# datasciencetoolkit/NextGP.jl

Measured on AMD Instinct MI355X. Metric: gibbs_iterations_per_sec, higher is better.
Workload: dtype f64; 1 GPU; single-trait Gibbs sweep, N=50000 individuals x P=600000 SNPs, marker sets BayesPR(200000) + BayesPR(200000) + BayesPR(200000), fp32 panel in HBM (BASELINE.json configs[3]: multi-breed random regression = three BayesPR marker sets of 200,000 SNPs); N=50000, P=600000, chains=1, panel_dtype=f32, accumulate_dtype=f64

## Files before the change

### nextgp.jl_amd/csrc/ngp_sweep.h

```cpp
#pragma once
#include <cstddef>
#include <type_traits>
#include "ngp_sweep_args.h"

#ifndef NGP_ROWS_DPP
#define NGP_ROWS_DPP 1
#endif

#pragma clang fp contract(off)

namespace ngp {


#define NGP_DBG_FOLD                                                     \
    unsigned long long *const dbg = DBG ? A.dbg : nullptr;               \
    const int dbg_mode = DBG ? A.dbg_mode : 0;                           \
    (void)dbg; (void)dbg_mode;
#define NGP_DBG_LOCALS                                                   \
    unsigned long long *const dbg = A.dbg;                               \
    const int dbg_mode = A.dbg_mode;                                     \
    (void)dbg; (void)dbg_mode;
#define NGP_DBG_ROWS NGP_DBG_FOLD

__device__ inline unsigned ld_u32(const unsigned *p) { return __hip_atomic_load(p, __ATOMIC_RELAXED, __HIP_MEMORY_SCOPE_AGENT); }
// ... 1051 lines not shown
                        red[(par * NGP_ROWS_NW + wv) * NGP_BLK + lane] = acc;
                        asm volatile("" ::: "memory");
                        if (lane == 0) __hip_atomic_fetch_add((lds_int_t *)(par ? gcnt1 : gcnt0), 1, __ATOMIC_RELAXED, __HIP_MEMORY_SCOPE_WORKGROUP);
                        try_signal(false);
                        const char *tq = ring + (size_t)wrap(base + tslot) * NGP_QS + c * 128;
#pragma unroll
                        for (int jj = 0; jj < 8; jj++) keep[d][hh][jj] = *(const float4 *)(tq + jj * 16);
                    }
                    if (wv == NGP_ROWS_PUBW && u < nb) {
                        const int *gc = par ? gcnt1 : gcnt0;
                        for (unsigned sp = 0; lds_flag_ld(gc) < NGP_ROWS_NW; ++sp) {
                            if ((sp & 255u) == 255u && (lds_flag_ld(sflag) == 0 || sp > (NGP_SPIN_LIMIT << 4))) {
                                if (lane == 0) *sflag = 0;
                                break;
                            }
                            __builtin_amdgcn_s_sleep(0);
                        }
                        asm volatile("" ::: "memory");
                        if (lane == 0) lds_flag_st(par ? gcnt0 : gcnt1, 0);
                        publish(u, hh, par);
                    }
                    if (pollw) {
                        int ok = 1;
                        if (!have_dnext) {
                            ok = wait_dlt_granules_all(A.dltg, A.nonce, pa, lane, A.abort_w, 1u, pg0, pg1) ? 1 : 0;
                            if (!ok && lane == 0) *sflag = 0;
                        }
                        if (ok) dl[((u + 1) & 1) * NGP_DLS + lane] = dlt_granules_value(pg0, pg1);
                    }
                    if (wv == NGP_ROWS_POLLW && hh == V - 1 && pa + 1 >= 0 && u + 2 < nb + DT) {
                        const unsigned long long *gp = A.dltg + ((size_t)((pa + 1) % NGP_RING) * NGP_BLK + lane) * 2;
                        pg0 = ld_u64(gp);
                        pg1 = ld_u64(gp + 1);
                    }
                    try_signal(DT < 4 || (A.knob & 16));
                    wg_barrier();
                    if (!*sflag) return;
                    base = wrap(base + NQ);
                }
            }
        }
        try_signal(true);
    }
    __syncthreads();
    for (int i = tid; i < V * R; i += NGP_WG) yg[i] = ys[(i / R) * RP + (i % R)];
}

template <bool DBG>
__device__ __attribute__((always_inline)) inline void role_reducer(const SweepArgs &A, const int g, char *smem, const int wv0 = 0,
                                                                   const int nwv = NGP_WG / 64) {
    NGP_DBG_LOCALS
    const int tid = threadIdx.x, wv = tid >> 6, lane = tid & 63;
    const int nb = A.t1 - A.t0;
    if (A.near + 1 + g >= A.D) return;
    const double fxs = A.scal->fx_scale;
    for (int u = wv - wv0; u < nb; u += nwv) {
        const int slot = u % NGP_RING;
        for (int d = A.near + 1 + g; d < A.D; d += A.NG) {
            const int a = u - d;
            if (a < 0) continue;
            double gr[NGP_BLK];
            load_rows_pair(A.gramx + ((size_t)(A.t0 + u) * A.D + d) * (NGP_BLK * NGP_BLK), lane, gr);
            unsigned long long q0, q1;
            {
                const unsigned long long *gp = A.dltg + ((size_t)(a % NGP_RING) * NGP_BLK + lane) * 2;
                q0 = ld_u64(gp);
                q1 = ld_u64(gp + 1);
            }
            if (!(dbg_mode == 3 || dbg_mode == 4 || dbg_mode == 6) && !wait_dlt_granules_all(A.dltg, A.nonce, a, lane, A.abort_w, 4u, q0, q1)) return;
            const double dreg = dlt_granules_value(q0, q1);
            double *ldw = (double *)smem + (size_t)wv * NGP_BLK;
            ldw[lane] = dreg;
            typedef const __attribute__((address_space(3))) double *lds_cdp;
            const lds_cdp dk = (lds_cdp)ldw;
            double s0 = 0.0, s1 = 0.0, s2 = 0.0, s3 = 0.0;
#pragma unroll
            for (int kk = 0; kk < NGP_BLK; kk += 16) {
                double dv[16];
#pragma unroll
                for (int i = 0; i < 16; i++) dv[i] = dk[kk + i];
#pragma unroll
                for (int i = 0; i < 16; i += 4) {
                    s0 = __builtin_fma(gr[kk + i + 0], dv[i + 0], s0);
                    s1 = __builtin_fma(gr[kk + i + 1], dv[i + 1], s1);
                    s2 = __builtin_fma(gr[kk + i + 2], dv[i + 2], s2);
                    s3 = __builtin_fma(gr[kk + i + 3], dv[i + 3], s3);
                }
                asm volatile("" : "+v"(s0), "+v"(s1), "+v"(s2), "+v"(s3));
            }
            const double v = (s0 + s1) + (s2 + s3);
            acc_add(A.acc, A.abort_w, slot, d, lane, -v, fxs);
            if (dbg && g == 0 && lane == 0) dbg[NGP_DBG_RED + 2 * (size_t)u + 1] = wall_clock64();
        }
    }
}

struct CoefRegs {
    double bo, cc, ww, st, gd;
    unsigned tf;
};
__device__ inline CoefRegs load_coef(const SweepArgs &A, long long k) {
    CoefRegs c;
    c.bo = A.beta[k];
    c.cc = A.c[k];
    c.ww = A.w[k];
    c.st = A.q[k];
    c.gd = A.mpm[k];
    c.tf = A.lin_all ? 1u : (A.blin ? A.blin[k >> 6] : 0u);
    return c;
}
__device__ __attribute__((always_inline)) inline unsigned acc_terms(const SweepArgs &A, const int u) {
    const int nfar = max(0, min(A.D - 1, u) - A.near);
    return (unsigned)(A.S + nfar);
}
__device__ __attribute__((always_inline)) inline unsigned long long acc_load(const SweepArgs &A, const int u, const int j) {
    const unsigned long long *ap = A.acc + (size_t)(u % NGP_RING) * NGP_FX_COPIES * NGP_BLK + j;
    unsigned long long qv[NGP_FX_COPIES];
#pragma unroll
    for (int c = 0; c < NGP_FX_COPIES; c++) qv[c] = ld_u64(ap + (size_t)c * NGP_BLK);
    unsigned long long q = qv[0];
#pragma unroll
    for (int c = 1; c < NGP_FX_COPIES; c++) q += qv[c];
    return q;
}
__device__ __attribute__((always_inline)) inline bool acc_complete(const unsigned long long q, const unsigned terms) {
    return __ballot((unsigned)(q & ((1ull << NGP_FX_CNT_BITS) - 1ull)) == terms) == ~0ull;
}
__device__ __attribute__((always_inline)) inline double acc_take(const SweepArgs &A, const int u, const int j, const unsigned long long q, const double fxi) {
    unsigned long long *ap = A.acc + (size_t)(u % NGP_RING) * NGP_FX_COPIES * NGP_BLK + j;
#pragma unroll
    for (int c = 0; c < NGP_FX_COPIES; c++) st_u64(ap + (size_t)c * NGP_BLK, 0ull);
    return fx_to_f64((long long)q >> NGP_FX_CNT_BITS) * fxi;
}
template <bool DBG, bool NGBIG = false>
__device__ __attribute__((always_inline)) inline bool fetch_group_sums(const SweepArgs &A, int u, int j, double *tot_out) {
    NGP_DBG_LOCALS
    const unsigned terms = acc_terms(A, u);
    const double fxi = A.scal->fx_inv;
    for (unsigned spins = 0;; ++spins) {
        const unsigned long long q = acc_load(A, u, j);
        if (dbg_mode == 2 || acc_complete(q, terms)) {
            *tot_out = acc_take(A, u, j, q, fxi);
            return true;
        }
        if ((spins & 7u) == 7u && ld_u32(A.abort_w) != 0u) return false;
        if (spins > (NGP_SPIN_LIMIT >> 3)) {
            st_u32(A.abort_w, 3u);
            return false;
        }
        __builtin_amdgcn_s_sleep(2);
    }
}

template <bool DBG>
__device__ __attribute__((always_inline)) inline void publish_block(const SweepArgs &A, int up, int j, const double *hist, const double *outb, const int *outi,
                                     const int *smeth, const double *ssdf) {
    NGP_DBG_LOCALS
    const int pbuf = up & 1;
    (void)hist;
    const long long k = (long long)(A.t0 + up) * NGP_BLK + j;
    const int si = A.setof[k];
    const double chik = A.chi[k];
    const int vbi = A.vbidx[k];
    st_f64(&A.dlt[(size_t)(up % NGP_RING) * NGP_BLK + j], hist[(up % NGP_RING) * NGP_BLK + j]);
    drain_vm();
    if (j == 0) st_u32(A.flag_dlt, (unsigned)(up + 1));
    if (dbg && j == 0) dbg[4 * (size_t)up + 2] = wall_clock64();
    const double bn = outb[pbuf * NGP_BLK + j];
    const int isave = outi[pbuf * NGP_BLK + j];
    A.beta[k] = bn;
    A.delta[k] = (uint8_t)isave;
    const int meth = (si >= 0) ? smeth[si] : -1;
    if (meth == 1) {
        double vb = 0.0;
        if (isave) {
            double tt = ssdf[si];
            double b2 = bn * bn;
            tt = tt + b2;
            vb = tt / chik;
            atomicAdd(&A.sets[si].nloci, 1);
        }
        A.varBeta[vbi] = vb;
    } else if (meth == 2) {
        if (isave) atomicAdd(&A.sets[si].nloci, 1);
    } else if (meth == 3) {
        atomicAdd(&A.sets[si].ncls[isave - 1], 1);
    }
}

struct RWide { double dmine; int c; };
__device__ __attribute__((noinline)) RWide rform_search_wide(const double *rcls, const size_t Ppad, const size_t col, const int j, const int Kk,
                                                             const double qv, const double av, const double tv, const double uv,
                                                             const double hs_k, const double rhs_k, const double bo_k) {
    const bool on = j < Kk;
    double q2 = qv, a2 = av, t2 = tv, u2 = uv;
    if (j >= NGP_RLDS && on) {
        const double *gp = rcls + (size_t)j * Ppad + col;
        const size_t gstr = (size_t)NGP_RMAX * Ppad;
        q2 = gp[0]; a2 = gp[gstr]; t2 = gp[2 * gstr]; u2 = gp[3 * gstr];
    }
    const double Lv = (q2 == 0.0) ? a2 : __builtin_fma(hs_k, q2, a2);
    RWide out;
    out.dmine = (q2 != 0.0) ? __builtin_fma(rhs_k, q2, t2) - bo_k : -bo_k;
    double m = readlane_d(Lv, 0);
#pragma unroll 1
    for (int v = 1; v < Kk; v++) {
        const double Lu = readlane_d(Lv, v);
        m = (Lu > m) ? Lu : m;
    }
    const double ev = on ? det_exp(Lv - m) : 0.0;
    double S = 0.0;
#pragma unroll 1
    for (int v = 0; v < Kk; v++) S = S + readlane_d(ev, v);
    int c = Kk - 1;
    double cum = 0.0;
#pragma unroll 1
    for (int v = 0; v < Kk; v++) {
        cum = cum + readlane_d(ev, v);
        const double thr = readlane_d(u2, v) * S;
        if (cum >= thr) { c = v; break; }
    }
    out.c = c;
    return out;
}

template <bool DBG, bool NGBIG = false, bool TUP = true, int RCLS = 1>
__device__ __attribute__((always_inline)) inline void role_sampler(const SweepArgs &A, char *smem) {
    NGP_DBG_LOCALS
    const int D = A.D, tid = threadIdx.x, wv = tid >> 6, j = tid & 63;
    double *Gd = (double *)smem;
    double *hist = Gd + 3 * 4096;
    double *vacc = hist + NGP_RING * NGP_BLK;
    double *r0 = vacc + NGP_RING * NGP_BLK;
    double *outb = r0 + 4 * NGP_BLK;
    int *outi = (int *)(outb + 2 * NGP_BLK);
    int *sabort = outi + 2 * NGP_BLK;
    int *totflag = sabort + 1;
    int *smeth = sabort + 4;
    double *ssdf = (double *)(sabort + 20);
    const int nb = A.t1 - A.t0;
    const size_t bsz = NGP_BLK * NGP_BLK;
    int *sK = sabort + 52;
    double *tl = (double *)(sabort + 80);
    int *tmeta = (int *)(tl + 2 * 9 * NGP_BLK);
    auto tuple_prefetch = [&](const int ub) __attribute__((always_inline)) {
        if (!TUP || !A.tup || ub >= nb) return;
        const long long tblk = (long long)(A.t0 + ub);
        const long long kcol = tblk * NGP_BLK + j;
        const int si = A.setof[kcol];
        const unsigned long long mask = __ballot(si >= 0 && smeth[si < 0 ? 0 : si] == NGP_METHOD_TUPLE_DEV);
        int *meta = tmeta + (ub & 1) * 4;
        if (mask == 0ull) {
            if (j == 0) meta[0] = 0;
            return;
        }
        const int sit = __builtin_amdgcn_readfirstlane(__shfl(si, __builtin_ctzll(mask)));
        const TupLane TL = load_tuplane(A.tupc, A.tupg, A.w, A.Ppad, kcol);
        const int k = A.tup[sit].k;
        const long long first_locus = (tblk - (A.tup[sit].col0 >> 6)) * tuple_loci_per_block(k);
        const int nvalid = tuple_nvalid(k, A.tup[sit].nloc, first_locus);
        double *dst = tl + (size_t)(ub & 1) * (9 * NGP_BLK) + j;
#pragma unroll
        for (int b = 0; b < NGP_KMAX; b++) { dst[b * NGP_BLK] = TL.crow[b]; dst[(NGP_KMAX + b) * NGP_BLK] = TL.grow[b]; }
        dst[2 * NGP_KMAX * NGP_BLK] = TL.ww;
        if (j == 0) { meta[0] = k; meta[1] = nvalid; }
    };
    double *rl = (double *)(tmeta + 16);
    int *rlm = (int *)(rl + 2 * 17 * NGP_BLK);
    int *rmeta = rlm + 2 * 128;
    double *rlx = (double *)(rmeta + 16);
    auto rcls_prefetch = [&](const int ub) __attribute__((always_inline)) {
        if (RCLS != 2 || !A.rcls || ub >= nb) return;
        const long long kcol = (long long)(A.t0 + ub) * NGP_BLK + j;
        const int si = A.setof[kcol];
        const int meth = (si >= 0) ? smeth[si] : -1;
        const int Kc = (si >= 0) ? sK[si] : 2;
        const unsigned long long mask = __ballot(meth == 3);
        if (j == 0) rmeta[(ub & 1) * 4] = (mask != 0ull) ? 1 : 0;
        if (mask == 0ull) return;
        RLane RL = empty_rlane();
        if (meth == 3) RL = load_rlane(A.rcls, A.Ppad, kcol, Kc, A.rhs0);
        double *dst = rl + (size_t)(ub & 1) * (17 * NGP_BLK) + j;
#pragma unroll
        for (int v = 0; v < NGP_RREG; v++) {
            dst[v * NGP_BLK] = RL.q[v]; dst[(4 + v) * NGP_BLK] = RL.a[v]; dst[(8 + v) * NGP_BLK] = RL.t[v]; dst[(12 + v) * NGP_BLK] = RL.u[v];
        }
        dst[16 * NGP_BLK] = RL.rhs0;
        rlm[(ub & 1) * 128 + j] = meth;
        rlm[(ub & 1) * 128 + 64 + j] = Kc;
        if (__ballot(meth == 3 && Kc > NGP_RREG) != 0ull) {
            double *dx = rlx + (size_t)(ub & 1) * (16 * NGP_BLK) + j;
#pragma unroll
            for (int arr = 0; arr < 4; arr++)
#pragma unroll
                for (int v = NGP_RREG; v < NGP_RLDS; v++) {
                    const bool on = (meth == 3) && v < Kc;
                    dx[(arr * 4 + v - NGP_RREG) * NGP_BLK] = on ? A.rcls[((size_t)arr * NGP_RMAX + v) * (size_t)A.Ppad + (size_t)kcol] : 0.0;
                }
        }
    };
    if (tid < 16) {
        smeth[tid] = A.sets[tid].method;
        ssdf[tid] = A.sets[tid].sdf;
        sK[tid] = A.sets[tid].K;
    }
    if (tid == 0) {
        *sabort = 0;
        *totflag = 0;
        st_u32(A.xcc_w, xcc_id() + 1u);
        if (dbg) { dbg[NGP_DBG_ALL - 2] = xcc_id(); dbg[NGP_DBG_ALL - 1] = (unsigned)__builtin_amdgcn_s_getreg((31 << 11) | 4); }
    }
    {
        const double *gd = chain_block_src(A, A.t0, A.lin_all || (A.blin && A.blin[A.t0] != 0u));
        for (int idx = tid; idx < 4096; idx += NGP_WG) Gd[idx] = gd[idx];
        if (nb > 1) {
            const double *gd1 = chain_block_src(A, A.t0 + 1, A.lin_all || (A.blin && A.blin[A.t0 + 1] != 0u));
            for (int idx = tid; idx < 4096; idx += NGP_WG) Gd[4096 + idx] = gd1[idx];
        }
    }
    __syncthreads();
    if (wv == 2) {
        double tot;
        if (fetch_group_sums<DBG, NGBIG>(A, 0, j, &tot)) r0[j] = tot;
        else if (j == 0) *sabort = 1;
    }
    if (wv == 1) { tuple_prefetch(0); rcls_prefetch(0); }
    __syncthreads();
    if (*sabort) return;
#define NGP_END_OF_BLOCK()                                                                       \
    do {                                                                                         \
        if (dbg && j == 0) dbg[NGP_DBG_WAVES + 8 * (size_t)u + wv] = wall_clock64();           \
        wg_barrier();                                                                            \
        if (*sabort) return;                                                                     \
    } while (0)
    if (wv == 0) {
        CoefRegs cur = load_coef(A, (long long)A.t0 * NGP_BLK + j), nxt = cur;
        double iVarE_sweep = 0.0;
        if constexpr (RCLS == 2) {
            if (A.rcls) iVarE_sweep = A.scal->iVarE;
        }
        for (int u = 0; u < nb; ++u) {
            const int t = A.t0 + u, buf = u & 1, slot = u % NGP_RING, rs = u & 3;
            if (dbg && j == 0) dbg[4 * (size_t)u] = wall_clock64();
            if (u + 1 < nb) nxt = load_coef(A, (long long)(t + 1) * NGP_BLK + j);
            constexpr bool PRELOAD = false;
            const bool tform = __builtin_amdgcn_readfirstlane((int)cur.tf) != 0;
            const double *gdb = Gd + (u % 3) * 4096 + j;
            double G[NGP_BLK];
            double tot;
            if (D == 1) {
                tot = r0[rs * NGP_BLK + j];
                bool okc = true;
                if (u >= 1) okc = fetch_group_sums<DBG, NGBIG>(A, u, j, &tot);
                if (!okc && j == 0) *sabort = 1;
            } else {
                for (unsigned sp = 0; lds_flag_ld(totflag) != u + 1; ++sp) {
                    if ((sp & 255u) == 255u && (lds_flag_ld(sabort) != 0 || sp > (NGP_SPIN_LIMIT << 4))) {
                        if (j == 0) *sabort = 1;
                        break;
                    }
                    __builtin_amdgcn_s_sleep(0);
                }
                asm volatile("" ::: "memory");
                tot = r0[rs * NGP_BLK + j];
            }
            if (DBG && dbg && j == 0) dbg[NGP_DBG_W5 + 4 * (size_t)u + 2] = wall_clock64();
            const double bo = cur.bo, cc = cur.cc, ww = cur.ww, st = cur.st;
            const double r = __builtin_fma(cur.gd, bo, tot);
#define NGP_LOAD_G()                                                           \
    if constexpr (!PRELOAD) { _Pragma("unroll") for (int kk = 0; kk < NGP_BLK; kk++) G[kk] = gdb[kk * NGP_BLK]; } \
    double H0 = -(cc * G[0]), H1 = -(cc * G[1]), H2 = -(cc * G[2]), H3 = -(cc * G[3]);
            double e = __builtin_fma(r, cc, ww);
            double dsave;
            int isave = 1;
            int meth0 = -1, si0 = -1, rblk = 0;
            if constexpr (RCLS == 1) {
                if (A.rcls) {
                    si0 = A.setof[(long long)t * NGP_BLK + j];
                    meth0 = (si0 >= 0) ? smeth[si0] : -1;
                }
            } else if constexpr (RCLS == 2) {
                if (A.rcls) rblk = __builtin_amdgcn_readfirstlane(rmeta[buf * 4]);
                if (rblk) meth0 = rlm[buf * 128 + j];
            }
            int tk = 0;
            if constexpr (TUP) {
                if (A.tup) tk = __builtin_amdgcn_readfirstlane(tmeta[buf * 4]);
            }
            if (tform && dbg_mode != 5) {
                double e0 = e;
                if constexpr (TUP) {
                    if (tk != 0) {
                        const int nvalid = __builtin_amdgcn_readfirstlane(tmeta[buf * 4 + 1]);
                        const double *tsrc = tl + (size_t)buf * (9 * NGP_BLK) + j;
                        TupLane TL;
#pragma unroll
                        for (int b = 0; b < NGP_KMAX; b++) { TL.crow[b] = tsrc[b * NGP_BLK]; TL.grow[b] = tsrc[(NGP_KMAX + b) * NGP_BLK]; }
                        TL.ww = tsrc[2 * NGP_KMAX * NGP_BLK];
                        e0 = tuple_e0(tk, nvalid, j, tot, bo, TL);
                    }
                }
                r0[rs * NGP_BLK + j] = e0;
                typedef const __attribute__((address_space(3))) double *lds_cdp;
                const lds_cdp ek = (lds_cdp)(r0 + rs * NGP_BLK);
                double s0 = 0.0, s1 = 0.0, s2 = 0.0, s3 = 0.0;
#pragma unroll
                for (int kk = 0; kk < NGP_BLK; kk += 16) {
                    double ev[16], tv[16];
#pragma unroll
                    for (int i = 0; i < 16; i++) ev[i] = ek[kk + i];
#pragma unroll
                    for (int i = 0; i < 16; i++) tv[i] = PRELOAD ? G[kk + i] : gdb[(kk + i) * NGP_BLK];
#pragma unroll
                    for (int i = 0; i < 16; i += 4) {
                        s0 = __builtin_fma(tv[i + 0], ev[i + 0], s0);
                        s1 = __builtin_fma(tv[i + 1], ev[i + 1], s1);
                        s2 = __builtin_fma(tv[i + 2], ev[i + 2], s2);
                        s3 = __builtin_fma(tv[i + 3], ev[i + 3], s3);
                    }
                    asm volatile("" : "+v"(s0), "+v"(s1), "+v"(s2), "+v"(s3));
                }
                dsave = (s0 + s1) + (s2 + s3);
                isave = 1;
            } else if (TUP && tk != 0) {
                const int nvalid = __builtin_amdgcn_readfirstlane(tmeta[buf * 4 + 1]);
                const double *tsrc = tl + (size_t)buf * (9 * NGP_BLK) + j;
                TupLane TL;
#pragma unroll
                for (int b = 0; b < NGP_KMAX; b++) { TL.crow[b] = tsrc[b * NGP_BLK]; TL.grow[b] = tsrc[(NGP_KMAX + b) * NGP_BLK]; }
                TL.ww = tsrc[2 * NGP_KMAX * NGP_BLK];
                dsave = tuple_chain_nv(tk, nvalid, j, tot, bo, TL, [&](int sl, int cc2) { return Gd[(u % 3) * 4096 + sl * NGP_BLK + cc2]; });
                isave = 1;
            } else if (RCLS != 0 && A.rcls && (RCLS == 2 ? rblk != 0 : __ballot(meth0 == 3) != 0ull)) {
                double dfin = 0.0;
                int cfin = 1;
                if constexpr (RCLS == 2) {
                    const double *cq = rl + (size_t)buf * (17 * NGP_BLK);
                    const double *cx = rlx + (size_t)buf * (16 * NGP_BLK);
                    const bool isr = (meth0 == 3);
                    const double q0j = cq[j], hstar = (isr && q0j == 0.0) ? cq[8 * NGP_BLK + j] : -1.0;
                    const double rhs0j = cq[16 * NGP_BLK + j];
                    const int Kj = rlm[buf * 128 + 64 + j];
                    const double iVarE = iVarE_sweep;
                    const int vj = (j < NGP_RLDS) ? j : 0;
                    const double *cls_base = (vj < NGP_RREG) ? cq + vj * NGP_BLK : cx + (vj - NGP_RREG) * NGP_BLK;
                    double rcur = r;
                    int kstart = 0;
                    for (int guard = 0; guard < NGP_BLK + 1; ++guard) {
                        double lazy_d, rhs = 0.0, hs = 0.0;
                        int lazy_c;
                        bool need;
                        if (isr) {
                            const double tt = rcur * iVarE;
                            rhs = tt + rhs0j;
                            const double s2 = rhs * rhs;
                            hs = 0.5 * s2;
                            need = (bo != 0.0) || !(hs <= hstar);
                            lazy_d = -bo;
                            lazy_c = 1;
                        } else {
                            eval_rform_other(rcur, bo, cc, ww, st, lazy_d, lazy_c);
                            need = (lazy_d != 0.0);
                        }
                        if (j >= kstart) { dfin = lazy_d; cfin = lazy_c; }
                        const unsigned long long todo = __ballot(need) & (~0ull << kstart);
                        if (!todo) break;
                        const int kk = __builtin_ctzll(todo);
                        const double Hk = -(gdb[kk * NGP_BLK]);
                        double dk;
                        if (__builtin_amdgcn_readlane(meth0, kk) == 3) {
                            const double rhs_k = readlane_d(rhs, kk), hs_k = readlane_d(hs, kk), bo_k = readlane_d(bo, kk);
                            const int Kk = __builtin_amdgcn_readlane(Kj, kk);
                            const bool on = j < Kk;
                            const double *cp = cls_base + kk;
                            const double qv = cp[0], av = cp[4 * NGP_BLK], tv = cp[8 * NGP_BLK], uv = cp[12 * NGP_BLK];
                            const double Lraw = (qv == 0.0) ? av : __builtin_fma(hs_k, qv, av);
                            const double dcls = __builtin_fma(rhs_k, qv, tv);
                            double dmine = (qv != 0.0) ? dcls - bo_k : -bo_k;
                            int c;
                            if (Kk <= NGP_RREG) {
                                const double Lv = on ? Lraw : -__builtin_inf();
                                const double up = on ? uv : __builtin_inf();
                                double m = __builtin_fmax(Lv, dpp_quad_f64<0xB1>(Lv));
                                m = __builtin_fmax(m, dpp_quad_f64<0x4E>(m));
                                const double ev = det_exp_le0(Lv - m);
                                const double c0 = dpp_quad_f64<0x00>(ev);
                                const double c1 = c0 + dpp_quad_f64<0x55>(ev);
                                const double c2 = c1 + dpp_quad_f64<0xAA>(ev);
                                const double c3 = c2 + dpp_quad_f64<0xFF>(ev);
                                const int vq = j & 3;
                                const double mycum = (vq == 0) ? c0 : ((vq == 1) ? c1 : ((vq == 2) ? c2 : c3));
                                const double thr = up * c3;
                                const unsigned hitm = (unsigned)__ballot(mycum >= thr) & 0xFu;
                                c = hitm ? __builtin_ctz(hitm) : Kk - 1;
                            } else if (Kk <= NGP_RLDS) {
                                const double Lv = Lraw;
                                double m = readlane_d(Lv, 0);
#pragma unroll
                                for (int v = 1; v < NGP_RLDS; v++) {
                                    if (v < Kk) {
                                        const double Lu = readlane_d(Lv, v);
                                        m = (Lu > m) ? Lu : m;
                                    }
                                }
                                const double ev = on ? det_exp(Lv - m) : 0.0;
                                double S = 0.0;
#pragma unroll
                                for (int v = 0; v < NGP_RLDS; v++)
                                    if (v < Kk) S = S + readlane_d(ev, v);
                                c = Kk - 1;
                                double cum = 0.0;
                                bool found = false;
#pragma unroll
                                for (int v = 0; v < NGP_RLDS; v++) {
                                    if (v < Kk && !found) {
                                        cum = cum + readlane_d(ev, v);
                                        const double thr = readlane_d(uv, v) * S;
                                        if (cum >= thr) { c = v; found = true; }
                                    }
                                }
                            } else {
                                const RWide rw = rform_search_wide(A.rcls, (size_t)A.Ppad, (size_t)((long long)t * NGP_BLK + kk), j, Kk, qv, av, tv, uv, hs_k, rhs_k, bo_k);
                                c = rw.c;
                                dmine = rw.dmine;
                            }
                            dk = readlane_d(dmine, c);
                            if (j == kk) { dfin = dk; cfin = c + 1; }
                        } else {
                            dk = readlane_d(lazy_d, kk);
                        }
                        if (dk != 0.0) rcur = __builtin_fma(Hk, dk, rcur);
                        kstart = kk + 1;
                        if (kstart >= NGP_BLK) break;
                    }
                } else {
                RLane RL = empty_rlane();
                double iVarE;
                {
                    if (meth0 == 3) RL = load_rlane(A.rcls, A.Ppad, (long long)t * NGP_BLK + j, sK[si0], A.rhs0);
                    iVarE = A.scal->iVarE;
                }
                double rcur = r;
                int kstart = 0;
                for (int guard = 0; guard < NGP_BLK + 1; ++guard) {
                    double cand;
                    int cls;
                    eval_rform(meth0, rcur, bo, cc, ww, st, RL, iVarE, cand, cls);
                    if (j >= kstart) { dfin = cand; cfin = cls; }
                    const unsigned long long todo = __ballot(cand != 0.0) & (~0ull << kstart);
                    if (!todo) break;
                    const int kk = __builtin_ctzll(todo);
                    const double dk = readlane_d(cand, kk);
                    const double Hk = -(gdb[kk * NGP_BLK]);
                    rcur = __builtin_fma(Hk, dk, rcur);
                    kstart = kk + 1;
                    if (kstart >= NGP_BLK) break;
                }
                }
                dsave = dfin;
                isave = cfin;
            } else if (dbg_mode == 5 && __ballot(st >= 0.0) == 0ull) {
                dsave = e;
            } else if (__ballot(st >= 0.0) == 0ull) {
                NGP_LOAD_G()
                if (DBG && dbg) {
                    asm volatile("s_waitcnt lgkmcnt(0)" ::: "memory");
                    if (j == 0) dbg[NGP_DBG_W5 + 4 * (size_t)u + 3] = wall_clock64();
                }
#pragma unroll
                for (int kk = 0; kk < NGP_BLK; kk += 4) {
                    double dk;
                    dk = readlane_d(e, kk + 0); e = __builtin_fma(H0, dk, e); H0 = -(cc * G[(kk + 4) & 63]);
                    dk = readlane_d(e, kk + 1); e = __builtin_fma(H1, dk, e); H1 = -(cc * G[(kk + 5) & 63]);
                    dk = readlane_d(e, kk + 2); e = __builtin_fma(H2, dk, e); H2 = -(cc * G[(kk + 6) & 63]);
                    dk = readlane_d(e, kk + 3); e = __builtin_fma(H3, dk, e); H3 = -(cc * G[(kk + 7) & 63]);
                }
                dsave = e;
            } else if (__popcll(__ballot((__builtin_fabs(r * cc) > st) || (bo != 0.0))) <= NGP_SPARSE_MAX) {
                double f = r * cc;
                const double nbo = -bo;
                unsigned long long todo = __ballot((__builtin_fabs(f) > st) || (bo != 0.0));
                while (todo) {
                    const int k = __builtin_ctzll(todo);
                    const double Hk = -(cc * gdb[k * NGP_BLK]);
                    const unsigned long long inm = __ballot(__builtin_fabs(f) > st);
                    const double ek = readlane_d(e, k), nk = readlane_d(nbo, k);
                    const double dk = ((inm >> k) & 1ull) ? ek : nk;
                    e = __builtin_fma(Hk, dk, e);
                    f = __builtin_fma(Hk, dk, f);
                    const unsigned long long later = (k == 63) ? 0ull : (~0ull << (k + 1));
                    todo = __ballot((__builtin_fabs(f) > st) || (bo != 0.0)) & later;
                }
                isave = __builtin_fabs(f) > st;
                dsave = isave ? e : -bo;
            } else {
                NGP_LOAD_G()
                double f = r * cc;
#pragma unroll
                for (int kk = 0; kk < NGP_BLK; kk += 4) {
#define NGP_STEP(HX, KO)                                              \
    {                                                                 \
        int in = __builtin_fabs(f) > st;                              \
        double dlv = in ? e : -bo;                                    \
        double dk = readlane_d(dlv, kk + KO);                         \
        e = __builtin_fma(HX, dk, e);                                 \
        f = __builtin_fma(HX, dk, f);                                 \
        HX = -(cc * G[(kk + KO + 4) & 63]);                           \
    }
                    NGP_STEP(H0, 0) NGP_STEP(H1, 1) NGP_STEP(H2, 2) NGP_STEP(H3, 3)
#undef NGP_STEP
                }
                isave = __builtin_fabs(f) > st;
                dsave = isave ? e : -bo;
            }
#undef NGP_LOAD_G
            hist[slot * NGP_BLK + j] = dsave;
            publish_dlt_granules(A.dltg, A.nonce, u, j, dsave);
            outb[buf * NGP_BLK + j] = bo + dsave;
            outi[buf * NGP_BLK + j] = isave;
            if (dbg && j == 0) dbg[4 * (size_t)u + 1] = wall_clock64();
            cur = nxt;
            NGP_END_OF_BLOCK();
        }
    } else if (wv == 1) {
        for (int u = 0; u < nb; ++u) {
            tuple_prefetch(u + 1);
            rcls_prefetch(u + 1);
            if (u >= 1) publish_block<DBG>(A, u - 1, j, hist, outb, outi, smeth, ssdf);
            NGP_END_OF_BLOCK();
        }
        if (nb >= 1) publish_block<DBG>(A, nb - 1, j, hist, outb, outi, smeth, ssdf);
    } else if (wv == 2) {
        if (D >= 4) {
            const double fxi = A.scal->fx_inv;
            unsigned long long qa = 0ull;
            int la = -1;
            int next_take = 1;
            if (nb > 1) {
                double tot1;
                if (fetch_group_sums<DBG, NGBIG>(A, 1, j, &tot1)) { r0[NGP_BLK + j] = tot1; next_take = 2; }
                else if (j == 0) *sabort = 1;
            }
            if (nb > 2) { qa = acc_load(A, 2, j); la = 2; }
            for (int u = 0; u < nb; ++u) {
                unsigned long long qn = 0ull;
                int ln = -1;
                {
                    const int want = (la >= 0 ? la : next_take - 1) + 1;
                    if (want < nb && want <= u + 3) { qn = acc_load(A, want, j); ln = want; }
                }
                if (next_take < nb && next_take <= u + 2) {
                    const bool must = (next_take == u + 1);
                    const unsigned terms = acc_terms(A, next_take);
                    unsigned long long q = qa;
                    bool ready = false;
                    int ok = 1;
                    if (la == next_take) ready = dbg_mode == 2 || acc_complete(q, terms);
                    else if (must || la < 0) { q = acc_load(A, next_take, j); ready = dbg_mode == 2 || acc_complete(q, terms); }
                    if (!ready && must) {
                        for (unsigned spins = 0;; ++spins) {
                            __builtin_amdgcn_s_sleep(2);
                            q = acc_load(A, next_take, j);
                            if (acc_complete(q, terms)) { ready = true; break; }
                            if ((spins & 7u) == 7u && ld_u32(A.abort_w) != 0u) { ok = 0; break; }
                            if (spins > (NGP_SPIN_LIMIT >> 3)) { st_u32(A.abort_w, 3u); ok = 0; break; }
                        }
                    }
                    if (!ok) {
                        if (j == 0) *sabort = 1;
                    } else if (ready) {
                        r0[(next_take & 3) * NGP_BLK + j] = acc_take(A, next_take, j, q, fxi);
                        if (dbg && j == 0) dbg[4 * (size_t)next_take + 3] = wall_clock64();
                        ++next_take;
                    }
                }
                if (ln == next_take) { qa = qn; la = ln; }
                else if (ln > next_take && ln >= 0) {
                    la = -1;
                    if (next_take < nb && next_take <= u + 3) { qa = acc_load(A, next_take, j); la = next_take; }
                } else la = -1;
                NGP_END_OF_BLOCK();
            }
        } else {
            for (int u = 0; u < nb; ++u) {
                if (u + 1 < nb && D >= 2) {
                    double tot;
                    if (fetch_group_sums<DBG, NGBIG>(A, u + 1, j, &tot)) r0[((u + 1) & 3) * NGP_BLK + j] = tot;
                    else if (j == 0) *sabort = 1;
                }
                NGP_END_OF_BLOCK();
            }
        }
    } else if (wv == 3) {
        const bool per_block = !A.lin_all && A.blin != nullptr;
        unsigned lin2 = A.lin_all ? 1u : 0u;
        if (per_block && nb > 2) lin2 = sld_u32(A.blin + A.t0 + 2);
        for (int u = 0; u < nb; ++u) {
            if (u + 2 < nb) {
                const char *gsrc = (const char *)chain_block_src(A, A.t0 + u + 2, lin2 != 0u) + (size_t)j * 16;
                char *gdst = (char *)(Gd + ((u + 2) % 3) * 4096);
#pragma unroll
                for (int i = 0; i < 32; i++)
                    __builtin_amdgcn_global_load_lds((const __attribute__((address_space(1))) void *)(gsrc + (size_t)i * 1024),
                                                     (__attribute__((address_space(3))) void *)(gdst + i * 1024), 16, 0, 0);
                asm volatile("s_waitcnt vmcnt(32)" ::: "memory");
            } else {
                drain_vm();
            }
            if (dbg && j == 0) dbg[NGP_DBG_WAVES + 8 * (size_t)u + wv] = wall_clock64();
            wg_barrier();
            unsigned ab;
            if (per_block && u + 3 < nb) sld_u32x2(A.abort_w, A.blin + A.t0 + u + 3, ab, lin2);
            else ab = sld_u32(A.abort_w);
            if (ab != 0u) return;
        }
    } else if (wv == 5) {
        double gxr[NGP_BLK];
#pragma unroll
        for (int kk = 0; kk < NGP_BLK; kk++) gxr[kk] = 0.0;
        for (int u = 0; u < nb; ++u) {
            if (D >= 2) {
                const int slot = u % NGP_RING, rs = u & 3;
                double tot = r0[rs * NGP_BLK + j];
                const bool have_far = (D >= 3) && (u >= 2) && (A.near >= 2);
                const bool have_one = (u >= 1);
                double cor = have_far ? vacc[slot * NGP_BLK + j] : 0.0;
                if (DBG && dbg) {
                    asm volatile("s_waitcnt vmcnt(0)" ::: "memory");
                    if (j == 0) dbg[NGP_DBG_W5 + 4 * (size_t)u] = wall_clock64();
                }
                if (have_one) {
                    typedef const __attribute__((address_space(3))) double *lds_cdp;
                    const lds_cdp dk = (lds_cdp)(hist + ((u - 1) % NGP_RING) * NGP_BLK);
                    double s0 = 0.0, s1 = 0.0, s2 = 0.0, s3 = 0.0;
#pragma unroll
                    for (int kk = 0; kk < NGP_BLK; kk += 16) {
                        double dv[16];
#pragma unroll
                        for (int i = 0; i < 16; i++) dv[i] = dk[kk + i];
#pragma unroll
                        for (int i = 0; i < 16; i += 4) {
                            s0 = __builtin_fma(gxr[kk + i + 0], dv[i + 0], s0);
                            s1 = __builtin_fma(gxr[kk + i + 1], dv[i + 1], s1);
                            s2 = __builtin_fma(gxr[kk + i + 2], dv[i + 2], s2);
                            s3 = __builtin_fma(gxr[kk + i + 3], dv[i + 3], s3);
                        }
                        asm volatile("" : "+v"(s0), "+v"(s1), "+v"(s2), "+v"(s3));
                    }
                    const double v1 = (s0 + s1) + (s2 + s3);
                    cor = have_far ? cor + v1 : v1;
                }
                if (have_far || have_one) tot = tot - cor;
                if (DBG && dbg && j == 0) dbg[NGP_DBG_W5 + 4 * (size_t)u + 1] = wall_clock64();
                r0[rs * NGP_BLK + j] = tot;
                asm volatile("s_waitcnt lgkmcnt(0)" ::: "memory");
                if (j == 0) lds_flag_st(totflag, u + 1);
                if (u + 1 < nb) {
                    load_rows_pair(A.gramx + ((size_t)(A.t0 + u + 1) * D + 1) * bsz, j, gxr);
                }
            }
            NGP_END_OF_BLOCK();
        }
    } else {
        const int fx = (wv == 4 && A.near >= 2) ? 2 : ((wv == 6 && A.near >= 3) ? 3 : (wv == 7 && A.near >= 4 ? 4 : 99));
        const int top = min(A.near, D - 1);
        double gr[NGP_BLK];
#pragma unroll
        for (int kk = 0; kk < NGP_BLK; kk++) gr[kk] = 0.0;
        bool have = false;
        for (int u = 0; u < nb; ++u) {
            if (fx < D) {
                if (u >= 1 && have) {
                    const int a = u - 1, upb = a + fx;
                    const double *dp = hist + (a % NGP_RING) * NGP_BLK;
                    double v = gemv4([&](int kk) { return gr[kk]; }, dp);
                    double *va = vacc + (upb % NGP_RING) * NGP_BLK + j;
                    const bool first = (fx == top) || (a == 0);
                    *va = first ? v : *va + v;
                }
                have = (u + fx < nb) && (u + 1 < nb);
                if (have) {
                    load_rows_pair(A.gramx + ((size_t)(A.t0 + u + fx) * D + fx) * bsz, j, gr);
                }
            }
            NGP_END_OF_BLOCK();
        }
    }
#undef NGP_END_OF_BLOCK
}

__device__ __attribute__((always_inline)) inline bool sweep_census(const SweepArgs &A, const int b, char *smem) {
    if (!A.census) return true;
    int *cflag = (int *)smem;
    if (threadIdx.x == 0) {
        A.census_tbl[b] = ((unsigned long long)(xcc_id() + 1u) << 32) | (unsigned)__builtin_amdgcn_s_getreg((31 << 11) | 4);
        if (A.census_fail != 0u && A.census_fail == A.iter_tag) atomicCAS(&A.census[1], 0u, 2u);
        const unsigned old = atomicAdd(&A.census[0], 1u);
        if (old + 1u == gridDim.x) atomicCAS(&A.census[1], 0u, 1u);
        const unsigned long long t0 = wall_clock64();
        unsigned verdict;
        while ((verdict = ld_u32(&A.census[1])) == 0u) {
            if (wall_clock64() - t0 > NGP_CENSUS_TICKS) atomicCAS(&A.census[1], 0u, 2u);
            else __builtin_amdgcn_s_sleep(8);
        }
        if (verdict != 1u) {
            st_u32(A.abort_w + 1, A.iter_tag);
            st_u32(A.abort_w, NGP_ABORT_CENSUS);
        }
        *cflag = (verdict == 1u) ? 1 : 0;
    }
    __syncthreads();
    const int cok = *cflag;
    __syncthreads();
    return cok != 0;
}

template <bool DBG>
__global__ __launch_bounds__(NGP_WG) __attribute__((amdgpu_waves_per_eu(2, 2))) void k_sweep(SweepArgs A) {
    constexpr bool TUP = DBG;
    constexpr int RCLSV = DBG ? 1 : 0;
#include "ngp_sweep_body.inc"
}
#if defined(NGP_INST_DBG) && NGP_INST_DBG == 2
__global__ __launch_bounds__(NGP_WG) __attribute__((amdgpu_waves_per_eu(2, 2))) void k_sweep_tup(SweepArgs A) {
    constexpr bool DBG = false, TUP = true;
    constexpr int RCLSV = 1;
#include "ngp_sweep_body.inc"
}
#endif
#if defined(NGP_INST_DBG) && NGP_INST_DBG == 3
__global__ __launch_bounds__(NGP_WG) __attribute__((amdgpu_waves_per_eu(2, 2))) void k_sweep_r(SweepArgs A) {
    constexpr bool DBG = false, TUP = true;
    constexpr int RCLSV = 2;
#include "ngp_sweep_body.inc"
}
#endif

#if defined(NGP_INST_DBG) && NGP_INST_DBG == 1
__global__ __launch_bounds__(NGP_WG) __attribute__((amdgpu_waves_per_eu(2, 2))) void k_sweep_tall(SweepArgs A) {
    extern __shared__ __attribute__((aligned(16))) char smem[];
    const int b = blockIdx.x;
    if (ld_u32(A.abort_w) != 0u) return;
    if (!sweep_census(A, b, smem)) return;
    if (b == 0)
        role_sampler<false, true>(A, smem);
    else if (b <= A.NG)
        role_reducer<false>(A, b - 1, smem);
    else if (A.V == 2)
        role_streamer_rows_tall<3, 2>(A, b - 1 - A.NG, smem);
    else
        role_streamer_rows_tall<2, 3>(A, b - 1 - A.NG, smem);
}
#endif

#ifndef NGP_MULTI_G
#define NGP_MULTI_G 4
#endif
template <int DT, int KC>
__device__ __attribute__((always_inline)) inline void role_streamer_multi(const MultiArgs &Mr, const int s, char *smem) {
    const MultiArgs *Mp = &Mr;
    const SweepArgs &A = Mp->a[0];
    static_assert(KC >= 2 && KC <= 8, "publication: waves 0-3, two chains each at most");
    const int R = A.R, S = A.S, tid = threadIdx.x;
    const int wv = __builtin_amdgcn_readfirstlane(tid >> 6), j = tid & 63;
    const size_t TBL = (size_t)(R >> 2) * NGP_QS;
    char *ring = smem;
    const size_t CH = ngp_multi_chain_doubles(R);
    double *cbase = (double *)(smem + 2 * TBL);
    int *sflag = (int *)(cbase + (size_t)KC * CH);
    char *scratch = (char *)sflag + 64;
#define NGP_YS(kc) (cbase + (size_t)(kc) * CH)
#define NGP_RED(kc) (NGP_YS(kc) + R)
#define NGP_DL(kc) (NGP_RED(kc) + 512)
#define NGP_PP(kc) (NGP_DL(kc) + 128)
    const size_t tile_elems = (size_t)R * NGP_BLK;
    const int nchunk = R >> 2;
    const int g = s / NGP_GRP;
    const int nb = A.t1 - A.t0;
    auto dma_tile = [&](int ub) {
        const char *src = (const char *)(A.tiles + ((size_t)(A.t0 + ub) * S + s) * tile_elems);
        char *dst = ring + (size_t)(ub & 1) * TBL;
        for (int c = wv - 4; c < nchunk; c += 3) dma16_lds(src + (size_t)c * 1024 + (size_t)j * 16, dst + (size_t)c * NGP_QS);
    };
    const double *dltp[KC];
    const unsigned *flagp[KC];
#pragma unroll
    for (int kc = 0; kc < KC; kc++) { dltp[kc] = Mp->a[kc].dlt; flagp[kc] = Mp->a[kc].flag_dlt; }
    const bool pubw = wv < 4 && wv < KC;
    const bool pub2 = pubw && (wv + 4 < KC);
    unsigned long long *my_acc = nullptr, *my_acc2 = nullptr;
    double my_fxs = 0.0, my_fxs2 = 0.0;
#pragma unroll
    for (int kc = 0; kc < KC; kc++) {
        if (kc == wv) { my_acc = Mp->a[kc].acc; my_fxs = Mp->a[kc].scal->fx_scale; }
        if (kc == wv + 4) { my_acc2 = Mp->a[kc].acc; my_fxs2 = Mp->a[kc].scal->fx_scale; }
    }
#pragma unroll
    for (int kc = 0; kc < KC; kc++) {
        const double *yg = Mp->a[kc].ycorr + (size_t)s * R;
        for (int i = tid; i < R; i += NGP_WG) NGP_YS(kc)[i] = yg[i];
    }
    if (tid == 0) *sflag = 1;
    auto wait_flags = [&](int target) -> int {
        int ok = 1;
#pragma unroll
        for (int kc = 0; kc < KC; kc++)
            if (j == kc) ok = wait_ge(flagp[kc], (unsigned)target, A.abort_w, 1u) ? 1 : 0;
        return __ballot(ok == 0) == 0ull ? 1 : 0;
    };
    auto poll_dlt = [&](int uu) {
        const int aa = uu - DT;
        if (aa < 0 || uu >= nb + DT) return;
        const int ok = wait_flags(aa + 1);
        if (!ok && j == 0) *sflag = 0;
        __builtin_amdgcn_fence(__ATOMIC_ACQUIRE, "wavefront");
        if (ok) {
            double v[KC];
#pragma unroll
            for (int kc = 0; kc < KC; kc++) v[kc] = ld_f64(&dltp[kc][(size_t)(aa % NGP_RING) * NGP_BLK + j]);
#pragma unroll
            for (int kc = 0; kc < KC; kc++) NGP_DL(kc)[(uu & 1) * 64 + j] = v[kc];
        }
    };
    const int tcc = wv, ti0 = min(j, R - 1);
    float keep[DT][8];
#pragma unroll
    for (int d = 0; d < DT; d++)
#pragma unroll
        for (int jj = 0; jj < 8; jj++) keep[d][jj] = 0.0f;
// ... 569 lines not shown
```

Measured before the change: 42.38 it/s.

## Stage per-block coefficients in LDS via publisher wave instead of sampler global loads

The sampler wave no longer loads the next block's coefficient registers from global memory. The publisher wave (wv 1) now loads coefficients two blocks ahead and writes them into a three-slot LDS staging ring, placed behind its vm drain, and the sampler reads its coefficients from LDS. To make room, the hist and vacc rings are re-partitioned with separate slot counts while r0 keeps its offset. The aim is to take global-load latency and register pressure off the serial sampler critical path. The cost is extra LDS traffic and reliance on barrier ordering between the waves.

Result: no change. 42.46 it/s (median of 2 runs) (+0.2%).

```diff
diff --git a/nextgp.jl_amd/csrc/ngp_sweep.h b/nextgp.jl_amd/csrc/ngp_sweep.h
--- a/nextgp.jl_amd/csrc/ngp_sweep.h
+++ b/nextgp.jl_amd/csrc/ngp_sweep.h
@@ -1227,9 +1227,17 @@
     }
 }
 
-template <bool DBG>
+#define NGP_HIST_SLOTS 4
+#define NGP_VACC_SLOTS 8
+#define NGP_COEF_SLOTS 3
+#define NGP_COEF_DOUBLES (5 * NGP_BLK)
+static_assert((NGP_HIST_SLOTS + NGP_VACC_SLOTS) * NGP_BLK + NGP_COEF_SLOTS * (NGP_COEF_DOUBLES + NGP_BLK / 2) <= 2 * NGP_RING * NGP_BLK,
+              "hist | vacc | staged coefficients | their flags must fit in front of r0");
+#define NGP_DBG_BAR (13u << 16)
+
+template <bool DBG, typename BehindDrain>
 __device__ __attribute__((always_inline)) inline void publish_block(const SweepArgs &A, int up, int j, const double *hist, const double *outb, const int *outi,
-                                     const int *smeth, const double *ssdf) {
+                                     const int *smeth, const double *ssdf, BehindDrain behind_drain) {
     NGP_DBG_LOCALS
     const int pbuf = up & 1;
     (void)hist;
@@ -1237,10 +1245,11 @@
     const int si = A.setof[k];
     const double chik = A.chi[k];
     const int vbi = A.vbidx[k];
-    st_f64(&A.dlt[(size_t)(up % NGP_RING) * NGP_BLK + j], hist[(up % NGP_RING) * NGP_BLK + j]);
+    st_f64(&A.dlt[(size_t)(up % NGP_RING) * NGP_BLK + j], hist[(up % NGP_HIST_SLOTS) * NGP_BLK + j]);
     drain_vm();
     if (j == 0) st_u32(A.flag_dlt, (unsigned)(up + 1));
     if (dbg && j == 0) dbg[4 * (size_t)up + 2] = wall_clock64();
+    behind_drain();
     const double bn = outb[pbuf * NGP_BLK + j];
     const int isave = outi[pbuf * NGP_BLK + j];
     A.beta[k] = bn;
@@ -1305,8 +1314,10 @@
     const int D = A.D, tid = threadIdx.x, wv = tid >> 6, j = tid & 63;
     double *Gd = (double *)smem;
     double *hist = Gd + 3 * 4096;
-    double *vacc = hist + NGP_RING * NGP_BLK;
-    double *r0 = vacc + NGP_RING * NGP_BLK;
+    double *vacc = hist + NGP_HIST_SLOTS * NGP_BLK;
+    double *cst = vacc + NGP_VACC_SLOTS * NGP_BLK;
+    int *ctf = (int *)(cst + NGP_COEF_SLOTS * NGP_COEF_DOUBLES);
+    double *r0 = hist + 2 * NGP_RING * NGP_BLK;
     double *outb = r0 + 4 * NGP_BLK;
     int *outi = (int *)(outb + 2 * NGP_BLK);
     int *sabort = outi + 2 * NGP_BLK;
@@ -1374,6 +1385,11 @@
                 }
         }
     };
+    auto coef_stage = [&](const int ub, const CoefRegs &cf) __attribute__((always_inline)) {
+        double *dst = cst + (ub % NGP_COEF_SLOTS) * NGP_COEF_DOUBLES + j;
+        dst[0] = cf.bo; dst[NGP_BLK] = cf.cc; dst[2 * NGP_BLK] = cf.ww; dst[3 * NGP_BLK] = cf.st; dst[4 * NGP_BLK] = cf.gd;
+        ctf[(ub % NGP_COEF_SLOTS) * NGP_BLK + j] = (int)cf.tf;
+    };
     if (tid < 16) {
         smeth[tid] = A.sets[tid].method;
         ssdf[tid] = A.sets[tid].sdf;
@@ -1399,7 +1415,11 @@
         if (fetch_group_sums<DBG, NGBIG>(A, 0, j, &tot)) r0[j] = tot;
         else if (j == 0) *sabort = 1;
     }
-    if (wv == 1) { tuple_prefetch(0); rcls_prefetch(0); }
+    if (wv == 1) {
+        tuple_prefetch(0); rcls_prefetch(0);
+        coef_stage(0, load_coef(A, (long long)A.t0 * NGP_BLK + j));
+        if (nb > 1) coef_stage(1, load_coef(A, (long long)(A.t0 + 1) * NGP_BLK + j));
+    }
     __syncthreads();
     if (*sabort) return;
 #define NGP_END_OF_BLOCK()                                                                       \
@@ -1409,15 +1429,19 @@
         if (*sabort) return;                                                                     \
     } while (0)
     if (wv == 0) {
-        CoefRegs cur = load_coef(A, (long long)A.t0 * NGP_BLK + j), nxt = cur;
         double iVarE_sweep = 0.0;
         if constexpr (RCLS == 2) {
             if (A.rcls) iVarE_sweep = A.scal->iVarE;
         }
         for (int u = 0; u < nb; ++u) {
-            const int t = A.t0 + u, buf = u & 1, slot = u % NGP_RING, rs = u & 3;
+            const int t = A.t0 + u, buf = u & 1, slot = u % NGP_HIST_SLOTS, rs = u & 3;
             if (dbg && j == 0) dbg[4 * (size_t)u] = wall_clock64();
-            if (u + 1 < nb) nxt = load_coef(A, (long long)(t + 1) * NGP_BLK + j);
+            CoefRegs cur;
+            {
+                const double *src = cst + (u % NGP_COEF_SLOTS) * NGP_COEF_DOUBLES + j;
+                cur.bo = src[0]; cur.cc = src[NGP_BLK]; cur.ww = src[2 * NGP_BLK]; cur.st = src[3 * NGP_BLK]; cur.gd = src[4 * NGP_BLK];
+                cur.tf = (unsigned)ctf[(u % NGP_COEF_SLOTS) * NGP_BLK + j];
+            }
             constexpr bool PRELOAD = false;
             const bool tform = __builtin_amdgcn_readfirstlane((int)cur.tf) != 0;
             const double *gdb = Gd + (u % 3) * 4096 + j;
@@ -1694,17 +1718,21 @@
             outb[buf * NGP_BLK + j] = bo + dsave;
             outi[buf * NGP_BLK + j] = isave;
             if (dbg && j == 0) dbg[4 * (size_t)u + 1] = wall_clock64();
-            cur = nxt;
-            NGP_END_OF_BLOCK();
+            if (dbg && j == 0) dbg[NGP_DBG_WAVES + 8 * (size_t)u + wv] = wall_clock64();
+            wg_barrier();
+            if (DBG && dbg && j == 0) dbg[NGP_DBG_BAR + (size_t)u + 1] = wall_clock64();
+            if (*sabort) return;
         }
     } else if (wv == 1) {
         for (int u = 0; u < nb; ++u) {
+            const CoefRegs ahead = load_coef(A, (long long)(A.t0 + min(u + 2, nb - 1)) * NGP_BLK + j);
             tuple_prefetch(u + 1);
             rcls_prefetch(u + 1);
-            if (u >= 1) publish_block<DBG>(A, u - 1, j, hist, outb, outi, smeth, ssdf);
+            if (u >= 1) publish_block<DBG>(A, u - 1, j, hist, outb, outi, smeth, ssdf, [&]() __attribute__((always_inline)) { coef_stage(u + 2, ahead); });
+            else coef_stage(2, ahead);
             NGP_END_OF_BLOCK();
         }
-        if (nb >= 1) publish_block<DBG>(A, nb - 1, j, hist, outb, outi, smeth, ssdf);
+        if (nb >= 1) publish_block<DBG>(A, nb - 1, j, hist, outb, outi, smeth, ssdf, []() {});
     } else if (wv == 2) {
         if (D >= 4) {
             const double fxi = A.scal->fx_inv;
@@ -1795,7 +1823,7 @@
         for (int kk = 0; kk < NGP_BLK; kk++) gxr[kk] = 0.0;
         for (int u = 0; u < nb; ++u) {
             if (D >= 2) {
-                const int slot = u % NGP_RING, rs = u & 3;
+                const int slot = u % NGP_VACC_SLOTS, rs = u & 3;
                 double tot = r0[rs * NGP_BLK + j];
                 const bool have_far = (D >= 3) && (u >= 2) && (A.near >= 2);
                 const bool have_one = (u >= 1);
@@ -1806,7 +1834,7 @@
                 }
                 if (have_one) {
                     typedef const __attribute__((address_space(3))) double *lds_cdp;
-                    const lds_cdp dk = (lds_cdp)(hist + ((u - 1) % NGP_RING) * NGP_BLK);
+                    const lds_cdp dk = (lds_cdp)(hist + ((u - 1) % NGP_HIST_SLOTS) * NGP_BLK);
                     double s0 = 0.0, s1 = 0.0, s2 = 0.0, s3 = 0.0;
 #pragma unroll
                     for (int kk = 0; kk < NGP_BLK; kk += 16) {
@@ -1847,9 +1875,9 @@
             if (fx < D) {
                 if (u >= 1 && have) {
                     const int a = u - 1, upb = a + fx;
-                    const double *dp = hist + (a % NGP_RING) * NGP_BLK;
+                    const double *dp = hist + (a % NGP_HIST_SLOTS) * NGP_BLK;
                     double v = gemv4([&](int kk) { return gr[kk]; }, dp);
-                    double *va = vacc + (upb % NGP_RING) * NGP_BLK + j;
+                    double *va = vacc + (upb % NGP_VACC_SLOTS) * NGP_BLK + j;
                     const bool first = (fx == top) || (a == 0);
                     *va = first ? v : *va + v;
                 }
```
